# fluent/chunkio

Measured on AMD Instinct MI355X. Metric: device-resident CRC32 GB/s over N×400KB chunks; % HBM-read roofline, higher is better.
Workload: dtype u8

## Files before the change

chunkio_amd/_lib.py:

```python
import ctypes
import os
import sys

HERE = os.path.dirname(os.path.abspath(__file__))
LIB_PATH = os.environ.get("CIO_AMD_LIB") or os.path.join(HERE, "lib", "libchunkio_amd.so")

EXPORTS = (
    "crc_update",
    "cio_gpu_init", "cio_gpu_last_error", "cio_gpu_version",
    "cio_crc32_shift", "cio_crc32_combine",
    "cio_crc32_plan_create", "cio_crc32_plan_destroy", "cio_crc32_plan_exec",
    "cio_crc32_plan_exec_events", "cio_crc32_plan_bytes", "cio_crc32_plan_kernel", "cio_crc32_plan_workgroups", "cio_crc32_ring_create", "cio_crc32_ring_exec",
    "cio_crc32_ring_join", "cio_crc32_ring_destroy", "cio_crc32_batch_dev", "cio_crc32_batch_host",
    "cio_crc32_devplan_create", "cio_crc32_devplan_destroy", "cio_crc32_devplan_exec", "cio_crc32_devplan_workgroups",
    "cio_crc32_batch_host_multi", "cio_crc32_split_host_multi", "cio_crc32_batch_fd_multi", "cio_gpu_device_count", "cio_gpu_set_device", "cio_gpu_get_device", "cio_gpu_numa_node",
    "cio_gpu_pci_bus_id", "cio_gpu_plan_cache_stats",
    "cio_crc32_host_register", "cio_crc32_host_unregister", "cio_gpu_pipe_last_timing",
    "cio_crc32_cpu_max", "cio_crc32_set_cpu_max", "cio_crc32_split_route", "cio_crc32_set_split_route", "cio_crc32_split_rates", "cio_crc32_split_forget", "cio_crc32_host_threads", "cio_crc32_set_host_threads",
    "cio_crc32_route_reset",
    "cio_crc32_batch_cpu", "cio_crc32_batch_fd_cpu",
    "cio_gpu_fill_synthetic", "cio_sha1_batch_dev", "cio_sha1_batch_dev_async",
    "cio_sha1_state_init", "cio_sha1_update_batch_dev", "cio_sha1_final_batch_dev", "cio_gpu_read_stream", "cio_gpu_read_stream_grid",
    "cio_gpu_event_create", "cio_gpu_event_destroy", "cio_gpu_event_record",
    "cio_gpu_event_elapsed_ms", "cio_gpu_stream_sync",
    "cio_sha1_init", "cio_sha1_update", "cio_sha1_final", "cio_sha1_hash", "cio_sha1_to_hex",
    "cioa_SHA1_Init", "cioa_SHA1_Update", "cioa_SHA1_Final",
    "cio_file_verify_batch", "cio_file_verify_batch_multi", "cio_verify_paths", "cio_verify_paths_multi",
    "cio_file_verify_batch_dev",
    "cio_dev_writer_create", "cio_dev_writer_destroy", "cio_file_init_batch_dev", "cio_file_write_batch_dev",
    "cio_file_seal_batch_dev",
    "cio_dev_writer_create_ex", "cio_dev_writer_move_segments", "cio_file_write_metadata_batch_dev",
    "cio_file_write_at_batch_dev",
    "cio_file_read_batch_dev", "cio_file_read_packed_batch_dev", "cio_meta_cmp_batch_dev",
    "cio_file_sync_batch", "cio_file_sync_batch_multi", "cio_file_sync_batch_begin", "cio_file_sync_batch_end",
    "cioa_create", "cioa_destroy", "cioa_set_max_chunks_up", "cioa_set_realloc_size_hint",
    "cioa_enable_file_trimming", "cioa_disable_file_trimming", "cioa_get_flags", "cioa_set_devices",
    "cioa_last_chunk_error", "cioa_total_chunks", "cioa_total_chunks_up",
    "cioa_stream_create", "cioa_stream_get", "cioa_stream_size_chunks_up", "cioa_stream_chunks", "cioa_scan_stream", "cioa_scan_streams", "cioa_scan_dump",
    "cioa_chunk_open", "cioa_chunk_close", "cioa_chunk_delete", "cioa_chunk_write", "cioa_chunk_write_at",
    "cioa_chunk_sync", "cioa_chunk_sync_batch", "cioa_chunk_sync_batch_begin", "cioa_chunk_sync_batch_end",
    "cioa_chunk_get_content", "cioa_chunk_get_content_copy",
    "cioa_chunk_get_content_size", "cioa_chunk_get_content_end_pos", "cioa_chunk_is_file",
    "cioa_chunk_close_stream", "cioa_chunk_get_real_size", "cioa_chunk_hash", "cioa_chunk_lock",
    "cioa_chunk_unlock", "cioa_chunk_is_locked", "cioa_chunk_tx_begin", "cioa_chunk_tx_commit",
    "cioa_chunk_tx_rollback", "cioa_chunk_is_up", "cioa_chunk_up", "cioa_chunk_up_force",
    "cioa_chunk_up_batch", "cioa_chunk_up_force_batch", "cioa_chunk_down",
    "cioa_chunk_name", "cioa_chunk_map", "cioa_error_get", "cioa_chunk_crc_cur", "cioa_chunk_set_crc_cur",
    "cioa_meta_write", "cioa_meta_read", "cioa_meta_cmp", "cioa_meta_size", "cioa_bench_perf_write",
)

_lib = None
_hip_runtime = None

c_u64_p = ctypes.POINTER(ctypes.c_uint64)
c_u32_p = ctypes.POINTER(ctypes.c_uint32)


def _bind(lib):
    V, P = ctypes.c_void_p, ctypes.POINTER
    sig = {
        "crc_update": (ctypes.c_uint64, [ctypes.c_uint64, V, ctypes.c_size_t]),
        "cio_gpu_init": (ctypes.c_int, []),
        "cio_gpu_last_error": (ctypes.c_char_p, []),
        "cio_gpu_version": (ctypes.c_char_p, []),
        "cio_crc32_shift": (ctypes.c_uint32, [ctypes.c_uint32, ctypes.c_uint64]),
        "cio_crc32_combine": (ctypes.c_uint32, [ctypes.c_uint32, ctypes.c_uint32, ctypes.c_uint64]),
        "cio_crc32_plan_create": (ctypes.c_int, [P(V), c_u64_p, c_u64_p, ctypes.c_size_t]),
        "cio_crc32_plan_destroy": (None, [V]),
        "cio_crc32_plan_exec": (ctypes.c_int, [V, V, V, V, V]),
        "cio_crc32_plan_exec_events": (ctypes.c_int, [V, V, V, V, V, V, V]),
        "cio_crc32_plan_bytes": (ctypes.c_uint64, [V]),
        "cio_crc32_plan_kernel": (ctypes.c_char_p, [V]),
        "cio_crc32_plan_workgroups": (ctypes.c_uint32, [V]),
        "cio_crc32_ring_create": (ctypes.c_int, [ctypes.POINTER(V), ctypes.POINTER(ctypes.c_uint64),
                                                 ctypes.POINTER(ctypes.c_uint64), ctypes.c_size_t, ctypes.c_int]),
        "cio_crc32_ring_exec": (ctypes.c_int, [V, V, V, V, V]),
        "cio_crc32_ring_join": (ctypes.c_int, [V, V]),
        "cio_crc32_ring_destroy": (None, [V]),
        "cio_crc32_batch_dev": (ctypes.c_int, [V, c_u64_p, c_u64_p, V, V, ctypes.c_size_t, V]),
        "cio_crc32_devplan_create": (ctypes.c_int, [P(V), ctypes.c_size_t]),
        "cio_crc32_devplan_destroy": (None, [V]),
        "cio_crc32_devplan_exec": (ctypes.c_int, [V, V, ctypes.c_uint64, V, V, ctypes.c_size_t, V, V, V, V]),
        "cio_crc32_devplan_workgroups": (ctypes.c_uint32, [V]),
        "cio_file_verify_batch_dev": (ctypes.c_int, [V, V, ctypes.c_uint64, V, V, ctypes.c_size_t, ctypes.c_int,
                                                     V, V, V, V, V, V]),
        "cio_dev_writer_create": (ctypes.c_int, [P(V), ctypes.c_size_t]),
        "cio_dev_writer_destroy": (None, [V]),
        "cio_file_init_batch_dev": (ctypes.c_int, [V, V, ctypes.c_uint64, V, V, ctypes.c_size_t, V, ctypes.c_uint64,
                                                   V, V, ctypes.c_int, V, V, V]),
        "cio_file_write_batch_dev": (ctypes.c_int, [V, V, ctypes.c_uint64, V, V, ctypes.c_size_t, V, ctypes.c_uint64,
                                                    V, V, ctypes.c_int, V, V, V]),
        "cio_file_seal_batch_dev": (ctypes.c_int, [V, V, ctypes.c_uint64, V, V, ctypes.c_size_t, ctypes.c_int,
                                                   V, V, V]),
        "cio_dev_writer_create_ex": (ctypes.c_int, [P(V), ctypes.c_size_t, ctypes.c_int]),
        "cio_dev_writer_move_segments": (ctypes.c_uint32, [V]),
        "cio_file_write_metadata_batch_dev": (ctypes.c_int, [V, V, ctypes.c_uint64, V, V, ctypes.c_size_t, V,
                                                             ctypes.c_uint64, V, V, ctypes.c_int, V, V, V]),
        "cio_file_write_at_batch_dev": (ctypes.c_int, [V, V, ctypes.c_uint64, V, V, ctypes.c_size_t, V, V,
                                                       ctypes.c_uint64, V, V, ctypes.c_int, V, V, V]),
        "cio_file_read_batch_dev": (ctypes.c_int, [V, V, ctypes.c_uint64, V, V, ctypes.c_size_t, ctypes.c_int, V,
                                                   V, ctypes.c_uint64, V, V, ctypes.c_int, V, V, V]),
        "cio_file_read_packed_batch_dev": (ctypes.c_int, [V, V, ctypes.c_uint64, V, V, ctypes.c_size_t, ctypes.c_int,
                                                          V, V, ctypes.c_uint64, ctypes.c_uint64, ctypes.c_int, V, V,
                                                          V, V, V]),
        "cio_meta_cmp_batch_dev": (ctypes.c_int, [V, ctypes.c_uint64, V, V, ctypes.c_size_t, V, ctypes.c_uint64, V,
                                                  V, V, V, V]),
        "cio_crc32_batch_host": (ctypes.c_int, [P(V), P(ctypes.c_size_t), c_u32_p, c_u32_p,
                                                ctypes.c_size_t]),
        "cio_crc32_batch_host_multi": (ctypes.c_int, [P(V), P(ctypes.c_size_t), c_u32_p, c_u32_p,
                                                      ctypes.c_size_t, P(ctypes.c_int), ctypes.c_int]),
        "cio_crc32_split_host_multi": (ctypes.c_int, [V, ctypes.c_size_t, ctypes.c_uint32, c_u32_p,
                                                      P(ctypes.c_int), ctypes.c_int]),
        "cio_gpu_device_count": (ctypes.c_int, []),
        "cio_gpu_set_device": (ctypes.c_int, [ctypes.c_int]),
        "cio_gpu_get_device": (ctypes.c_int, []),
        "cio_gpu_numa_node": (ctypes.c_int, [ctypes.c_int]),
        "cio_gpu_pci_bus_id": (ctypes.c_int, [ctypes.c_int, ctypes.c_char_p, ctypes.c_int]),
        "cio_gpu_plan_cache_stats": (ctypes.c_int, [ctypes.POINTER(ctypes.c_uint64), ctypes.c_int]),
        "cio_crc32_host_register": (ctypes.c_int, [V, ctypes.c_size_t]),
        "cio_crc32_host_unregister": (ctypes.c_int, [V]),
        "cio_gpu_pipe_last_timing": (ctypes.c_int, [P(ctypes.c_double), ctypes.c_int]),
        "cio_crc32_cpu_max": (ctypes.c_size_t, []),
        "cio_crc32_set_cpu_max": (None, [ctypes.c_size_t]),
        "cio_crc32_split_route": (ctypes.c_int, []),
        "cio_crc32_set_split_route": (None, [ctypes.c_int]),
        "cio_crc32_split_rates": (None, [ctypes.POINTER(ctypes.c_double), ctypes.c_int]),
# ... 116 lines not shown
```

chunkio_amd/crc32.py:

```python
import ctypes

import numpy as np

from . import _lib

CRC_INIT = 0xFFFFFFFF


def crc_init():
    return CRC_INIT


def crc_finalize(crc):
    return (crc ^ 0xFFFFFFFF) & 0xFFFFFFFF


def _as_bytes(data):
    if isinstance(data, np.ndarray):
        return np.ascontiguousarray(data).view(np.uint8)
    return np.frombuffer(memoryview(data).cast("B"), dtype=np.uint8)


def crc_update(crc, data):
    buf = _as_bytes(data)
# ... 2 lines not shown


def crc32(data, seed=CRC_INIT):
    return crc_finalize(crc_update(seed, data))


def crc32_shift(raw_state, nbytes):
    return int(_lib.lib().cio_crc32_shift(raw_state & 0xFFFFFFFF, nbytes))


def crc32_combine(raw_a, raw0_b, len_b):
    return int(_lib.lib().cio_crc32_combine(raw_a & 0xFFFFFFFF, raw0_b & 0xFFFFFFFF, len_b))


def _u64_array(values):
    arr = np.ascontiguousarray(np.asarray(values, dtype=np.uint64))
    return arr, arr.ctypes.data_as(_lib.c_u64_p)


def _ptr(t):
    return None if t is None else ctypes.c_void_p(t.data_ptr())


def _stream_ptr(stream):
    if stream is None:
        import torch
        stream = torch.cuda.current_stream()
    return ctypes.c_void_p(int(stream.cuda_stream))


class Crc32Plan:

    def __init__(self, offs, lens):
        self._offs, po = _u64_array(offs)
        self._lens, pl = _u64_array(lens)
        if self._offs.shape != self._lens.shape:
            raise ValueError("offs and lens must have the same length")
        self.n = int(self._offs.size)
        handle = ctypes.c_void_p()
        _lib.check(_lib.lib().cio_crc32_plan_create(ctypes.byref(handle), po, pl, self.n),
                   "cio_crc32_plan_create")
        self._handle = handle

    @property
    def bytes(self):
        return int(_lib.lib().cio_crc32_plan_bytes(self._handle))

    @property
    def workgroups(self):
        return int(_lib.lib().cio_crc32_plan_workgroups(self._handle))

    def kernel_name(self):
        return _lib.lib().cio_crc32_plan_kernel(self._handle).decode()

    def exec(self, base, out, seeds=None, stream=None):
        _lib.check(_lib.lib().cio_crc32_plan_exec(self._handle, _ptr(base), _ptr(seeds), _ptr(out),
                                                  _stream_ptr(stream)),
                   "cio_crc32_plan_exec")

    def exec_events(self, base, out, ev_start, ev_stop, seeds=None, stream=None):
        _lib.check(_lib.lib().cio_crc32_plan_exec_events(self._handle, _ptr(base), _ptr(seeds),
                                                         _ptr(out), _stream_ptr(stream),
                                                         ev_start, ev_stop),
                   "cio_crc32_plan_exec_events")

    def close(self):
        if getattr(self, "_handle", None):
            _lib.lib().cio_crc32_plan_destroy(self._handle)
            self._handle = None

    def __del__(self):
        try:
            self.close()
        except Exception:
            pass

    def __enter__(self):
        return self

    def __exit__(self, *exc):
        self.close()


class Crc32Ring:

    def __init__(self, offs, lens, depth=2):
        self._offs, po = _u64_array(offs)
        self._lens, pl = _u64_array(lens)
        if self._offs.shape != self._lens.shape:
            raise ValueError("offs and lens must have the same length")
        self.n = int(self._offs.size)
        handle = ctypes.c_void_p()
        _lib.check(_lib.lib().cio_crc32_ring_create(ctypes.byref(handle), po, pl, self.n, int(depth)),
                   "cio_crc32_ring_create")
        self._handle = handle

    def exec(self, base, out, seeds=None, stream=None):
        _lib.check(_lib.lib().cio_crc32_ring_exec(self._handle, _ptr(base), _ptr(seeds), _ptr(out),
                                                  _stream_ptr(stream)),
                   "cio_crc32_ring_exec")

    def join(self, stream=None):
        _lib.check(_lib.lib().cio_crc32_ring_join(self._handle, _stream_ptr(stream)), "cio_crc32_ring_join")

    def close(self):
        if getattr(self, "_handle", None):
# ... 334 lines not shown
```

chunkio_amd/csrc/cio_plan.h:

```cpp
#ifndef CIOA_PLAN_H
#define CIOA_PLAN_H

#include <stddef.h>
#include <stdint.h>
#include <vector>

#include "cio_diag.h"
#include "crc32_host.h"
#include "chunkio_amd/cio_crc32_gpu.h"

namespace cioa {

constexpr int kWave = 64;
constexpr int kGran = 16;
constexpr int kSub = 4;
constexpr int kRow = kWave * kGran;
constexpr int kStep = kSub * kRow;
constexpr int kThreads = 1024;
constexpr uint32_t kWavesPerWg = kThreads / kWave;
constexpr uint32_t kWfFold = 1u, kWfPublish = 2u;
constexpr int kX8Count = 2 * kStep;
constexpr uint32_t kSliceBytes = 131072;
constexpr uint32_t kShiftBytes = 32768;
constexpr uint32_t kShiftOff = kSliceBytes;
constexpr uint32_t kLdsBytes = kSliceBytes + kShiftBytes;
constexpr int kStampWords = 16;

struct ChunkDesc {
    uint64_t a;
    uint64_t vlen;
    uint64_t g;
    uint32_t nsteps;
    uint32_t h;
    uint32_t npieces;
    uint32_t w0, w1;
    uint32_t pad;
};
static_assert(sizeof(ChunkDesc) == 48, "desc layout");

struct WaveStart {
    ChunkDesc d;
    uint32_t c;
    uint32_t pad[3];
};
static_assert(sizeof(WaveStart) == 64, "wave start layout");

struct DeviceState {
    bool ready = false;
    int cus = 0;
    uint32_t *slice = nullptr;
    uint32_t *shift = nullptr;
    uint32_t *x8 = nullptr;
    uint32_t *xinv8 = nullptr;
};

struct PlanHost {
    std::vector<ChunkDesc> desc;
    std::vector<WaveStart> ws;
    std::vector<uint32_t> tiny;
    std::vector<uint32_t> pfac;
    uint64_t S = 0, bytes = 0;
};

void plan_init(cio_crc32_plan *p, DeviceState *st, size_t n);
const char *plan_build(PlanHost &ph, const uint64_t *offs, const uint64_t *lens, size_t n, uint32_t W);
const char *plan_choose(cio_crc32_plan *p, PlanHost &ph, const uint64_t *offs, const uint64_t *lens, size_t n);

constexpr int kDevHdrS = 0, kDevHdrNtiny = 1, kDevHdrBytes = 2, kDevHdrStatus = 3, kDevHdrWords = 4;
constexpr uint32_t kPlanBlock = 1024;

struct PlanBlockSum {
    uint64_t steps, bytes;
    uint32_t ntiny, err;
};

}

struct cio_crc32_plan {
    uint32_t n = 0;
    uint64_t S = 0;
    uint32_t W = 0;
    uint32_t grid = 0;
    uint32_t ntiny = 0;
    int prio = 1;
    uint64_t ustride = 0, ua0 = 0, uvlen = 0;
    uint32_t unsteps = 0, uh = 0;
    bool small = false;
    bool ahead = false;
    bool l64 = false;
    bool l64_small = false;
    unsigned long long *stamps = nullptr;
    uint64_t bytes = 0;
    cioa::ChunkDesc *desc = nullptr;
    cioa::WaveStart *wstart = nullptr;
    uint32_t *tiny = nullptr;
    unsigned long long *partials = nullptr;
    uint32_t *counters = nullptr;
    uint32_t *pfac = nullptr;
    cioa::DeviceState *st = nullptr;
};

#endif
```

chunkio_amd/csrc/crc32_gpu.hip:

```cpp

#include <hip/hip_runtime.h>
#include <stdint.h>
#include <algorithm>
#include <type_traits>

#include "cio_gpu_internal.h"
#include "crc_wave.h"

using namespace cioa;

namespace {


constexpr uint32_t cx_multmodp(uint32_t a, uint32_t b)
{
    uint32_t p = 0;
    for (int i = 31; i >= 0; --i) {
        if ((a >> i) & 1u) {
            p ^= b;
        }
        b = (b & 1u) ? (b >> 1) ^ CIOA_POLY : (b >> 1);
    }
    return p;
}
// ... 782 lines not shown
        t_arrived = __builtin_amdgcn_s_memrealtime();
    }
    tiny_chunks(lds, lb_lo, base, desc, tiny, seeds, out, cid, ntiny, wave, lane, W);
    __syncthreads();
    if (STAMPS) {
        t_bar1 = __builtin_amdgcn_s_memrealtime();
    }
    uint32_t *slot = reinterpret_cast<uint32_t *>(lds);
    if (lane == 0) {
        slot[tid >> 6] = pub;
    }
    __syncthreads();
    if (STAMPS) {
        t_bar2 = __builtin_amdgcn_s_memrealtime();
    }
    if (wfl & kWfFold) {
        const uint32_t nb = (wfl >> 8) & 0xffu;
        uint32_t a = 0;
        if (lane < kWavesPerWg && lane >= kWavesPerWg - nb) {
            a = slot[(tid >> 6) + lane - kWavesPerWg];
        }
        a = wave_xor(a) ^ fold_own;
        if (lane == 0) {
            out[cid ? cid[c0] : c0] = a;
        }
    }
    if (STAMPS) {
        t_folded = __builtin_amdgcn_s_memrealtime();
    }
    if (STAMPS && lane == 0) {
        uint32_t hw_id, xcc_id;
        asm volatile("s_getreg_b32 %0, hwreg(HW_REG_HW_ID)" : "=s"(hw_id));
        asm volatile("s_getreg_b32 %0, hwreg(HW_REG_XCC_ID)" : "=s"(xcc_id));
        stamps[kStampWords * wave + 0] = t_entry;
        stamps[kStampWords * wave + 1] = t_tables;
        stamps[kStampWords * wave + 2] = t_stream;
        stamps[kStampWords * wave + 3] = __builtin_amdgcn_s_memrealtime();
        stamps[kStampWords * wave + 4] = hw_id;
        stamps[kStampWords * wave + 5] = xcc_id;
        stamps[kStampWords * wave + 6] = t_first;
        stamps[kStampWords * wave + 7] = t_mid;
        stamps[kStampWords * wave + 8] = t_issued;
        stamps[kStampWords * wave + 9] = t_wt[0];
        stamps[kStampWords * wave + 10] = t_wt[1];
        stamps[kStampWords * wave + 11] = t_step1;
        stamps[kStampWords * wave + 12] = t_arrived;
        stamps[kStampWords * wave + 13] = t_bar1;
        stamps[kStampWords * wave + 14] = t_bar2;
        stamps[kStampWords * wave + 15] = t_folded;
    }
}


struct SmallRegs {
    uint4 q[kSub];
    uint32_t inv;
    uint32_t seed;
};

__device__ __forceinline__ uint4 mask_tail(uint4 v, uint32_t bs, uint32_t vlen)
{
    uint32_t w[4] = {v.x, v.y, v.z, v.w};
#pragma unroll
    for (int i = 0; i < 4; ++i) {
        const uint32_t b = bs + 4u * i;
        const uint32_t nb = b >= vlen ? 0u : min(vlen - b, 4u);
        w[i] &= nb >= 4u ? ~0u : ((1u << (8u * nb)) - 1u);
    }
    return make_uint4(w[0], w[1], w[2], w[3]);
}

template <bool UNI, bool SEEDS, bool L64 = false>
__global__ void __launch_bounds__(kThreads, 1)
crc32_small_kernel(const uint8_t *base, uint64_t ustride, uint64_t ua0, uint64_t uvlen, uint32_t uh,
                   uint32_t W, uint32_t n, uint32_t ntiny, const uint32_t *__restrict__ g_x8,
                   const ChunkDesc *__restrict__ desc,
                   const uint32_t *__restrict__ tiny, const uint32_t *__restrict__ seeds, uint32_t *out,
                   const uint32_t *__restrict__ g_xinv8)
{
    __shared__ __attribute__((aligned(16))) char lds[kLdsBytes];
    const uint32_t tid = threadIdx.x;
    const uint32_t wave = __builtin_amdgcn_readfirstlane(blockIdx.x * (kThreads / kWave) + (tid >> 6));
    const uint32_t lane = tid & 63u;
    const uint32_t lb_lo = (lane & kSliceRepMask) << 2;
    const uint32_t lb_hi = lb_lo | 0x10000u;
    const uint32_t lrep = (lane & kShiftRepMask) << 2;
    const uint32_t c0 = __builtin_amdgcn_readfirstlane((uint32_t) split_point(wave, n, W));
    const uint32_t c1 = __builtin_amdgcn_readfirstlane((uint32_t) split_point((uint64_t) wave + 1, n, W));
    const uint32_t lbyte = lane * kGran;
    const uint32_t loff = L64 ? 64u * (lane & 15u) + 16u * (lane >> 4) : lbyte;
    const uint32_t *const seeds_p = seeds ? seeds : g_x8;

    auto geom = [&](uint32_t c, uint64_t &a, uint32_t &vlen, uint32_t &h, bool &live) {
        if (UNI) {
            a = ua0 + (uint64_t) c * ustride;
            vlen = (uint32_t) uvlen;
            h = uh;
            asm volatile("" : "+s"(vlen), "+s"(h));
            live = true;
        } else {
            const ChunkDesc d = desc[c];
            a = d.a;
            vlen = (uint32_t) d.vlen;
            h = d.h;
            live = d.nsteps != 0;
        }
// ... 95 lines not shown
            }
            st = block16(lds, lb_lo, lb_hi, 0u, r.q[0]);
#pragma unroll
            for (int q = 1; q < kSub; ++q) {
                st = L64 ? block16(lds, lb_lo, lb_hi, st, r.q[q])
                         : shift_block16(lds, lb_lo, lb_hi, lrep, st, r.q[q]);
            }
        }
        uint32_t inv = inv_u;
        if (!UNI) {
            asm volatile("v_mov_b32 %0, %1" : "=v"(inv) : "v"(cur.inv));
        }
        issue(cur, c + 1);
        if (live) {
            uint32_t x = col[0] & (0u - (st & 1u));
#pragma unroll
            for (int j = 1; j < 32; ++j) {
                x = xor_and(x, 0u - ((st >> j) & 1u), col[j]);
            }
            uint32_t crc = wave_xor(x);
            if (vlen != (uint32_t) kStep) {
                asm volatile("" : "+v"(inv));
                crc = multmodp(inv, crc);
            }
            if (lane == 0) {
                out[c] = crc;
            }
        }
    };
    const uint32_t slot_group = __builtin_amdgcn_readfirstlane((tid >> 6) >> 2);
    for (uint32_t c = c0; c < c1; ++c) {
        rotate_prio(slot_group, c - c0);
        chunk(cur, c);
    }
    __builtin_amdgcn_s_setprio(0);
    tiny_chunks(lds, lb_lo, base, desc, tiny, seeds, out, nullptr, ntiny, wave, lane, W);
}


}

extern "C" {

int cioa_debug_stamps(const cio_crc32_plan *p, unsigned long long *host, size_t cap)
{
    if (!p || !p->stamps) {
        return 0;
    }
    const size_t n = std::min(cap, (size_t) p->W * kStampWords);
    if (hipMemcpy(host, p->stamps, n * sizeof(unsigned long long), hipMemcpyDeviceToHost) != hipSuccess) {
        return 0;
    }
    return (int) p->W;
}

}

using StreamKernel = decltype(&crc32_stream_kernel<false, 1, false>);

static StreamKernel select_kernel(int prio, bool stamps, bool uniform, bool ahead, bool l64)
{
    if (ahead) {
        if (l64) {
            if (stamps) {
                return crc32_stream_kernel<true, 1, true, true, true>;
            }
            return prio ? crc32_stream_kernel<false, 1, true, true, true>
                        : crc32_stream_kernel<false, 0, true, true, true>;
        }
        return prio ? crc32_stream_kernel<false, 1, true, true> : crc32_stream_kernel<false, 0, true, true>;
    }
    if (l64 && !stamps) {
        return prio ? crc32_stream_kernel<false, 1, false, false, true>
                    : crc32_stream_kernel<false, 0, false, false, true>;
    }
    switch ((prio ? 4 : 0) + (stamps ? 2 : 0) + (uniform ? 1 : 0)) {
    case 0: return crc32_stream_kernel<false, 0, false>;
    case 1: return crc32_stream_kernel<false, 0, true>;
    case 2: return crc32_stream_kernel<true, 0, false>;
    case 3: return crc32_stream_kernel<true, 0, true>;
    case 4: return crc32_stream_kernel<false, 1, false>;
    case 5: return crc32_stream_kernel<false, 1, true>;
    case 6: return crc32_stream_kernel<true, 1, false>;
    default: return crc32_stream_kernel<true, 1, true>;
    }
}


int cioa::plan_exec_impl(const cio_crc32_plan *p, const void *dev_base, const uint32_t *dev_seeds,
                         uint32_t *dev_out, const uint32_t *cid, hipStream_t s,
                         hipEvent_t ev0, hipEvent_t ev1)
{
    if (!p) {
        return fail("cio_crc32_plan_exec: null plan");
    }
    if (p->n == 0) {
        return CIO_OK;
    }
    if (!dev_base || !dev_out) {
        return fail("cio_crc32_plan_exec: null buffer");
    }
    const DeviceState *st = p->st;
    if (ev0) {
        HIP_TRY(hipEventRecord(ev0, s), "hipEventRecord");
    }
    if (p->small && !cid) {
        auto sk = p->l64_small ? (p->unsteps ? (dev_seeds ? crc32_small_kernel<true, true, true>
                                                    : crc32_small_kernel<true, false, true>)
                                       : (dev_seeds ? crc32_small_kernel<false, true, true>
                                                    : crc32_small_kernel<false, false, true>))
                         : (p->unsteps ? (dev_seeds ? crc32_small_kernel<true, true> : crc32_small_kernel<true, false>)
                                       : (dev_seeds ? crc32_small_kernel<false, true>
                                                    : crc32_small_kernel<false, false>));
        hipLaunchKernelGGL(sk, dim3(p->grid), dim3(kThreads), 0, s,
                           reinterpret_cast<const uint8_t *>(dev_base), p->ustride, p->ua0, p->uvlen, p->uh,
                           p->W, p->n, p->ntiny, st->x8, p->desc, p->tiny, dev_seeds, dev_out, st->xinv8);
        HIP_TRY(hipGetLastError(), "crc32_small_kernel launch");
        if (ev1) {
            HIP_TRY(hipEventRecord(ev1, s), "hipEventRecord");
        }
        return CIO_OK;
    }
    auto kern = select_kernel(p->prio, p->stamps != nullptr, p->unsteps != 0, p->ahead && (!p->stamps || p->l64),
                              p->l64);
    hipLaunchKernelGGL(kern, dim3(p->grid), dim3(kThreads), 0, s,
                       reinterpret_cast<const uint8_t *>(dev_base), p->S, p->ustride, p->ua0, p->uvlen,
                       p->W, p->unsteps, p->uh, p->n, p->desc, p->wstart, p->tiny,
                       dev_seeds, dev_out, cid, p->partials, p->counters, st->slice, st->shift,
                       st->x8, p->pfac, p->ntiny, p->stamps);
    HIP_TRY(hipGetLastError(), "crc32_stream_kernel launch");
    if (ev1) {
        HIP_TRY(hipEventRecord(ev1, s), "hipEventRecord");
    }
    return CIO_OK;
}

int cioa::devplan_crc_launch(const cio_crc32_plan *p, const unsigned long long *hdr, const void *dev_base,
                             const uint32_t *dev_seeds, uint32_t *dev_out, size_t n, hipStream_t s)
{
    const DeviceState *st = p->st;
    StreamKernel kern = p->l64 ? (p->prio ? crc32_stream_kernel<false, 1, false, false, true, true>
                                          : crc32_stream_kernel<false, 0, false, false, true, true>)
                               : (p->prio ? crc32_stream_kernel<false, 1, false, false, false, true>
                                          : crc32_stream_kernel<false, 0, false, false, false, true>);
    hipLaunchKernelGGL(kern, dim3(p->grid), dim3(kThreads), 0, s,
                       reinterpret_cast<const uint8_t *>(dev_base), (uint64_t) 0, (uint64_t) 0, (uint64_t) 0,
                       (uint64_t) 0, p->W, 0u, 0u, (uint32_t) n, p->desc, p->wstart, p->tiny,
                       dev_seeds, dev_out, (const uint32_t *) nullptr, p->partials, p->counters, st->slice,
                       st->shift, st->x8, p->pfac, 0u, const_cast<unsigned long long *>(hdr));
    HIP_TRY(hipGetLastError(), "crc32_stream_kernel (device-planned) launch");
    return CIO_OK;
}
```

chunkio_amd/csrc/crc_plan.cpp:

```cpp

#include <stdint.h>
#include <stdlib.h>
#include <string.h>
#include <algorithm>
#include <vector>

#include "cio_plan.h"

namespace cioa {

void plan_init(cio_crc32_plan *p, DeviceState *st, size_t n)
{
    p->st = st;
    p->n = (uint32_t) n;
    if (const char *r = cioa_diag_getenv("CIO_GPU_PRIO")) {
        const int v = atoi(r);
        p->prio = (v == 0) ? 0 : 1;
    }
    p->l64 = true;
    p->l64_small = false;
    if (const char *r = cioa_diag_getenv("CIO_GPU_L64")) {
        p->l64 = p->l64_small = atoi(r) != 0;
    }
    p->grid = (uint32_t) st->cus;
// ... 148 lines not shown
    p->uh = ph.desc[0].h;
    p->unsteps = ph.desc[0].nsteps;
}

}

const char *plan_choose(cio_crc32_plan *p, PlanHost &ph, const uint64_t *offs, const uint64_t *lens, size_t n)
{
    if (const char *err = plan_build(ph, offs, lens, n, p->W)) {
        return err;
    }
    plan_uniform(p, offs, lens, n, ph);
    auto small_batch = [&ph, n] { return ph.S > 0 && ph.S == (uint64_t) n - ph.tiny.size(); };
    bool oversub = false;
    if (!cioa_diag_getenv("CIO_GPU_GRID") && ph.S >= 1024ull * p->W && 4ull * p->W <= 65536 &&
        !small_batch()) {
        PlanHost ph4;
        if (plan_build(ph4, offs, lens, n, 4 * p->W) == nullptr) {
            p->grid *= 4;
            p->W *= 4;
            oversub = true;
            ph = std::move(ph4);
        }
    }
    {
        const char *r = cioa_diag_getenv("CIO_GPU_ANTICAMP");
        const bool on = !(r && atoi(r) == 0);
        const char *mx = cioa_diag_getenv("CIO_GPU_ANTICAMP_MAX");
        const uint64_t wmax = mx ? strtoull(mx, nullptr, 10) : small_batch() ? 128 : 64;
        const uint64_t w = p->W ? ph.S / p->W : 0;
        const bool any_grid = r && atoi(r) == 2;
        if (on && (!oversub || any_grid) && !cioa_diag_getenv("CIO_GPU_GRID") && p->grid % 32 == 0 && ph.S % p->W == 0 &&
            w % 16 == 0 &&
            w > 0 && w <= wmax) {
            const uint32_t g2 = p->grid / 32 * 31;
            PlanHost ph2;
            if (plan_build(ph2, offs, lens, n, g2 * (kThreads / kWave)) == nullptr) {
                p->grid = g2;
                p->W = g2 * (kThreads / kWave);
                ph = std::move(ph2);
            }
        }
    }
    p->S = ph.S;
    p->bytes = ph.bytes;
    p->ntiny = (uint32_t) ph.tiny.size();
    p->ahead = p->unsteps != 0 && p->uh == 0 && p->uvlen % kStep == 0;
    bool short_ranges = p->S <= 64ull * p->W;
    if (const char *r = cioa_diag_getenv("CIO_GPU_AHEAD")) {
        short_ranges = atoi(r) != 0;
    }
    p->ahead = p->ahead && short_ranges;

    p->small = small_batch();
    if (const char *r = cioa_diag_getenv("CIO_GPU_SMALL")) {
        p->small = p->small && atoi(r) != 0;
    }
    return nullptr;
}

}

using namespace cioa;

extern "C" {

int cioa_debug_plan_layout(const uint64_t *offs, const uint64_t *lens, size_t n, uint32_t W,
                           uint32_t *chunk_words, uint32_t *wave_flags)
{
    PlanHost ph;
    if (plan_build(ph, offs, lens, n, W) != nullptr) {
        return -1;
    }
    for (size_t i = 0; i < n; i++) {
        chunk_words[3 * i + 0] = ph.desc[i].w0;
        chunk_words[3 * i + 1] = ph.desc[i].w1;
        chunk_words[3 * i + 2] = ph.desc[i].npieces;
    }
    const size_t nslots = (size_t) W + n + 1;
    for (uint32_t w = 0; w < W; w++) {
        wave_flags[w] = ph.pfac[nslots + w];
    }
    return 0;
}

int cioa_debug_plan_image(const uint64_t *offs, const uint64_t *lens, size_t n, uint32_t W, void *desc,
                          void *wstart, uint32_t *tiny, uint32_t *pfac, uint64_t *hdr)
{
    PlanHost ph;
    if (plan_build(ph, offs, lens, n, W) != nullptr) {
        return -1;
    }
    memcpy(desc, ph.desc.data(), n * sizeof(ChunkDesc));
    memcpy(wstart, ph.ws.data(), (size_t) W * sizeof(WaveStart));
    if (!ph.tiny.empty()) {
        memcpy(tiny, ph.tiny.data(), ph.tiny.size() * sizeof(uint32_t));
    }
    memcpy(pfac, ph.pfac.data(), ph.pfac.size() * sizeof(uint32_t));
    hdr[kDevHdrS] = ph.S;
    hdr[kDevHdrNtiny] = ph.tiny.size();
    hdr[kDevHdrBytes] = ph.bytes;
    hdr[kDevHdrStatus] = 0;
    return 0;
}

int cioa_debug_plan_choice(const uint64_t *offs, const uint64_t *lens, size_t n, int cus, uint32_t *out_words)
{
    if (cus < 1 || n >= 0xffffffffull) {
        return -1;
    }
    DeviceState st;
    st.cus = cus;
    cio_crc32_plan p;
    PlanHost ph;
    plan_init(&p, &st, n);
    if (plan_choose(&p, ph, offs, lens, n) != nullptr) {
        return -1;
    }
    const uint64_t ntiny = p.ntiny;
    const uint32_t words[11] = {p.grid, p.W, p.small, p.ahead, p.unsteps, p.l64, p.l64_small,
                                (uint32_t) p.S, (uint32_t) (p.S >> 32), (uint32_t) ntiny, (uint32_t) (ntiny >> 32)};
    memcpy(out_words, words, sizeof(words));
    return 0;
}

}
```

chunkio_amd/csrc/gpu_runtime.hip:

```cpp

#include <hip/hip_runtime.h>
#include <stdint.h>
#include <string.h>
#include <stdio.h>
#include <stdlib.h>
#include <memory>
#include <mutex>
#include <vector>
#include <string>
#include <algorithm>

#include "cio_gpu_internal.h"

using namespace cioa;

namespace cioa {

thread_local std::string g_err;

int fail(const char *what, hipError_t e)
{
    char buf[512];
    if (e != hipSuccess) {
        snprintf(buf, sizeof(buf), "%s: %s", what, hipGetErrorString(e));
// ... 32 lines not shown
    if (!st.ready) {
        hipDeviceProp_t prop;
        HIP_TRY(hipGetDeviceProperties(&prop, dev), "hipGetDeviceProperties");
        if (strncmp(prop.gcnArchName, "gfx950", 6) != 0) {
            char msg[256];
            snprintf(msg, sizeof(msg), "chunkio_amd kernels are built for gfx950, device is %s",
                     prop.gcnArchName);
            return fail(msg);
        }
        st.cus = prop.multiProcessorCount;
        static uint32_t slice[4][256], shift[4][256];
        std::vector<uint32_t> x8(kX8Count);
        cioa_gen_slice4(slice);
        cioa_gen_shift_table(shift, (uint64_t) (kStep - kGran));
        cioa_gen_xpow8_table(x8.data(), kX8Count, 1);
        HIP_TRY(hipMalloc(&st.slice, sizeof(slice)), "hipMalloc(slice)");
        HIP_TRY(hipMalloc(&st.shift, sizeof(shift)), "hipMalloc(shift)");
        HIP_TRY(hipMalloc(&st.x8, kX8Count * sizeof(uint32_t)), "hipMalloc(x8)");
        HIP_TRY(hipMemcpy(st.slice, slice, sizeof(slice), hipMemcpyHostToDevice), "upload slice");
        HIP_TRY(hipMemcpy(st.shift, shift, sizeof(shift), hipMemcpyHostToDevice), "upload shift");
        HIP_TRY(hipMemcpy(st.x8, x8.data(), kX8Count * sizeof(uint32_t), hipMemcpyHostToDevice),
                "upload x8");
        std::vector<uint32_t> xinv8(kStep);
        uint32_t xm8 = 0x80000000u;
        for (int i = 0; i < 8; ++i) {
            xm8 = cioa_multmodp(xm8, (CIOA_POLY << 1) | 1u);
        }
        xinv8[0] = 0x80000000u;
        for (int d = 1; d < kStep; ++d) {
            xinv8[d] = cioa_multmodp(xinv8[d - 1], xm8);
        }
        HIP_TRY(hipMalloc(&st.xinv8, kStep * sizeof(uint32_t)), "hipMalloc(xinv8)");
        HIP_TRY(hipMemcpy(st.xinv8, xinv8.data(), kStep * sizeof(uint32_t), hipMemcpyHostToDevice),
                "upload xinv8");
        st.ready = true;
    }
    *out = &st;
    return CIO_OK;
}

}

extern "C" {

const char *cio_gpu_last_error(void)
{
    return g_err.c_str();
}

const char *cio_gpu_version(void)
{
#define CIO_STR2(x) #x
#define CIO_STR(x) CIO_STR2(x)
    return "chunkio_amd crc32 v9 gfx950 stream(l64-lanes permlane-transpose issue-ahead<=64steps pre-shift prio-rotate "
           "coalesced-nt division-free-start slice4-lds32x perm direct-whole preshifted-partials wg-lds-fold "
           "head-align=" CIO_STR(CIO_HEAD_ALIGN) ") "
           "small(4x16B dpp-reduce bitop3-fold prio-rotate) "
           "host(nt-staging graduated-groups pread-bounce multi-device vpclmul-crc_update small-batch-route) "
           "sha1(2-schedule-waves 4-block-handover continuation)";
}

int cio_gpu_init(void)
{
    DeviceState *st;
    return device_state(&st);
}

void cio_crc32_plan_destroy(cio_crc32_plan *p)
{
    if (!p) {
        return;
    }
    (void) hipFree(p->desc);
    (void) hipFree(p->wstart);
    (void) hipFree(p->tiny);
    (void) hipFree(p->partials);
    (void) hipFree(p->counters);
    (void) hipFree(p->pfac);
    (void) hipFree(p->stamps);
    delete p;
}

int cio_crc32_plan_create(cio_crc32_plan **out, const uint64_t *offs, const uint64_t *lens, size_t n)
{
    if (!out || (n && (!offs || !lens))) {
        return fail("cio_crc32_plan_create: null argument");
    }
    if (n >= 0xffffffffull) {
        return fail("cio_crc32_plan_create: too many chunks");
    }
    *out = nullptr;
    DeviceState *st;
    if (device_state(&st) != CIO_OK) {
        return CIO_ERROR;
    }
    cio_crc32_plan *p = new cio_crc32_plan();
    plan_init(p, st, n);
    PlanHost ph;
    if (const char *err = plan_choose(p, ph, offs, lens, n)) {
        delete p;
        return fail(err);
    }
    if (const char *r = cioa_diag_getenv("CIO_GPU_STAMPS")) {
        if (atoi(r) > 0 && hipMalloc(&p->stamps, (size_t) p->W * kStampWords * sizeof(unsigned long long)) != hipSuccess) {
            p->stamps = nullptr;
        }
    }
    hipError_t e;
    const size_t npart = ph.pfac.size();
    if ((e = hipMalloc(&p->desc, ph.desc.size() * sizeof(ChunkDesc))) != hipSuccess ||
        (e = hipMalloc(&p->wstart, ph.ws.size() * sizeof(WaveStart))) != hipSuccess ||
        (e = hipMalloc(&p->tiny, std::max<size_t>(1, ph.tiny.size()) * sizeof(uint32_t))) != hipSuccess ||
        (e = hipMalloc(&p->partials, npart * sizeof(unsigned long long))) != hipSuccess ||
        (e = hipMalloc(&p->counters, std::max<size_t>(1, n) * sizeof(uint32_t))) != hipSuccess ||
        (e = hipMalloc(&p->pfac, npart * sizeof(uint32_t))) != hipSuccess ||
        (e = hipMemcpy(p->desc, ph.desc.data(), ph.desc.size() * sizeof(ChunkDesc), hipMemcpyHostToDevice)) != hipSuccess ||
        (e = hipMemcpy(p->wstart, ph.ws.data(), ph.ws.size() * sizeof(WaveStart), hipMemcpyHostToDevice)) != hipSuccess ||
        (ph.tiny.size() && (e = hipMemcpy(p->tiny, ph.tiny.data(), ph.tiny.size() * sizeof(uint32_t), hipMemcpyHostToDevice)) != hipSuccess) ||
        (e = hipMemset(p->partials, 0, npart * sizeof(unsigned long long))) != hipSuccess ||
        (e = hipMemset(p->counters, 0, std::max<size_t>(1, n) * sizeof(uint32_t))) != hipSuccess ||
        (e = hipMemcpy(p->pfac, ph.pfac.data(), npart * sizeof(uint32_t), hipMemcpyHostToDevice)) != hipSuccess) {
        cio_crc32_plan_destroy(p);
        return fail("cio_crc32_plan_create: device allocation/upload", e);
    }
    *out = p;
    return CIO_OK;
}

uint64_t cio_crc32_plan_bytes(const cio_crc32_plan *p)
{
    return p ? p->bytes : 0;
}

uint32_t cio_crc32_plan_workgroups(const cio_crc32_plan *p)
{
    return p ? p->grid : 0;
}

const char *cio_crc32_plan_kernel(const cio_crc32_plan *p)
{
    return (p && p->small) ? "crc32_small_kernel" : "crc32_stream_kernel";
}

int cio_crc32_plan_exec_events(const cio_crc32_plan *p, const void *dev_base,
                               const uint32_t *dev_seeds, uint32_t *dev_out, void *stream,
                               void *ev_piece_start, void *ev_piece_stop)
{
    return plan_exec_impl(p, dev_base, dev_seeds, dev_out, nullptr,
                          reinterpret_cast<hipStream_t>(stream),
                          reinterpret_cast<hipEvent_t>(ev_piece_start),
                          reinterpret_cast<hipEvent_t>(ev_piece_stop));
}

int cio_crc32_plan_exec(const cio_crc32_plan *p, const void *dev_base, const uint32_t *dev_seeds,
                        uint32_t *dev_out, void *stream)
{
    return plan_exec_impl(p, dev_base, dev_seeds, dev_out, nullptr,
                          reinterpret_cast<hipStream_t>(stream));
}

int cio_crc32_batch_dev(const void *dev_base, const uint64_t *offs, const uint64_t *lens,
                        const uint32_t *dev_seeds, uint32_t *dev_out, size_t n, void *stream)
{
    cio_crc32_plan *p = nullptr;
    if (cio_crc32_plan_create(&p, offs, lens, n) != CIO_OK) {
        return CIO_ERROR;
    }
    int rc = cio_crc32_plan_exec(p, dev_base, dev_seeds, dev_out, stream);
    if (rc == CIO_OK) {
        hipError_t e = hipStreamSynchronize(reinterpret_cast<hipStream_t>(stream));
        if (e != hipSuccess) {
            rc = fail("cio_crc32_batch_dev: stream sync", e);
        }
    }
    cio_crc32_plan_destroy(p);
    return rc;
}

struct cio_crc32_ring {
    std::vector<cio_crc32_plan *> plans;
    std::vector<hipStream_t> streams;
    std::vector<hipEvent_t> ready, done;
    std::vector<bool> pending;
    unsigned next = 0;
    int dev = 0;
};

struct RingDevice {
    int prev = -1;
    hipError_t e = hipSuccess;
    explicit RingDevice(int dev)
    {
        if ((e = hipGetDevice(&prev)) == hipSuccess && prev != dev) {
            e = hipSetDevice(dev);
// ... 146 lines not shown
```

include/chunkio_amd/cio_crc32_gpu.h:

```cpp
#ifndef CIO_CRC32_GPU_H
#define CIO_CRC32_GPU_H

#include <stddef.h>
#include <stdint.h>
#include <chunkio_amd/cio_sha1_state.h>

#ifdef __cplusplus
extern "C" {
#endif

#ifndef CIO_OK
#define CIO_OK       0
#define CIO_ERROR   -1
#endif


int cio_gpu_init(void);

int cio_gpu_device_count(void);
int cio_gpu_set_device(int dev);
int cio_gpu_get_device(void);

int cio_gpu_numa_node(int dev);

int cio_gpu_pci_bus_id(int dev, char *buf, int len);

const char *cio_gpu_last_error(void);

const char *cio_gpu_version(void);


uint32_t cio_crc32_shift(uint32_t raw_state, uint64_t nbytes);

uint32_t cio_crc32_combine(uint32_t raw_a, uint32_t raw0_b, uint64_t len_b);


typedef struct cio_crc32_plan cio_crc32_plan;

int  cio_crc32_plan_create(cio_crc32_plan **plan, const uint64_t *offs,
                           const uint64_t *lens, size_t n);
void cio_crc32_plan_destroy(cio_crc32_plan *plan);

int  cio_crc32_plan_exec(const cio_crc32_plan *plan, const void *dev_base,
                         const uint32_t *dev_seeds, uint32_t *dev_out,
                         void *stream);

int  cio_crc32_plan_exec_events(const cio_crc32_plan *plan, const void *dev_base,
                                const uint32_t *dev_seeds, uint32_t *dev_out,
                                void *stream, void *ev_piece_start,
                                void *ev_piece_stop);

uint64_t cio_crc32_plan_bytes(const cio_crc32_plan *plan);

const char *cio_crc32_plan_kernel(const cio_crc32_plan *plan);

typedef struct cio_crc32_ring cio_crc32_ring;
int  cio_crc32_ring_create(cio_crc32_ring **ring, const uint64_t *offs, const uint64_t *lens, size_t n, int depth);
int  cio_crc32_ring_exec(cio_crc32_ring *ring, const void *dev_base, const uint32_t *dev_seeds, uint32_t *dev_out,
                         void *stream);
int  cio_crc32_ring_join(cio_crc32_ring *ring, void *stream);
void cio_crc32_ring_destroy(cio_crc32_ring *ring);

uint32_t cio_crc32_plan_workgroups(const cio_crc32_plan *plan);

int  cio_crc32_batch_dev(const void *dev_base, const uint64_t *offs,
                         const uint64_t *lens, const uint32_t *dev_seeds,
                         uint32_t *dev_out, size_t n, void *stream);

typedef struct cio_crc32_devplan cio_crc32_devplan;

#define CIO_DEVPLAN_E_BOUNDS           1
#define CIO_DEVPLAN_E_CHUNK_TOO_LARGE  2
#define CIO_DEVPLAN_E_BATCH_TOO_LARGE  4

int  cio_crc32_devplan_create(cio_crc32_devplan **plan, size_t max_chunks);
void cio_crc32_devplan_destroy(cio_crc32_devplan *plan);

int  cio_crc32_devplan_exec(cio_crc32_devplan *plan, const void *dev_base, uint64_t dev_bytes,
                            const uint64_t *dev_offs, const uint64_t *dev_lens, size_t n,
                            const uint32_t *dev_seeds, uint32_t *dev_out,
                            uint32_t *dev_status, void *stream);

uint32_t cio_crc32_devplan_workgroups(const cio_crc32_devplan *plan);


int  cio_crc32_batch_host(const void *const *bufs, const size_t *lens,
                          const uint32_t *seeds, uint32_t *out_raw, size_t n);

int  cio_crc32_batch_host_multi(const void *const *bufs, const size_t *lens,
                                const uint32_t *seeds, uint32_t *out_raw, size_t n,
                                const int *devices, int ndev);

int  cio_crc32_split_host_multi(const void *buf, size_t len, uint32_t seed, uint32_t *out_raw,
                                const int *devices, int ndev);

int  cio_crc32_batch_fd_multi(const int *fds, const uint64_t *foffs, const size_t *lens,
                              const uint32_t *seeds, uint32_t *out_raw, size_t n,
                              const int *devices, int ndev);

int  cio_crc32_host_register(const void *p, size_t len);
int  cio_crc32_host_unregister(const void *p);

int  cio_gpu_pipe_last_timing(double *out, int n);

int  cio_gpu_plan_cache_stats(uint64_t *out, int n);


// ... 60 lines not shown
```

Before: 6289.

## Add wave-aligned CRC32 kernel for uniform chunk layouts with precomputed shift factors

Adds a specialized kernel used when every chunk splits evenly into a power-of-two number of wave pieces with equal step counts. Each wave derives its chunk and piece from its index, so it skips the generic per-wave start descriptors. It combines partial CRCs with precomputed per-lane shift factors through an LDS fold within the workgroup instead of global partials and counters. The path is on by default when the plan's conditions hold and adds a separate factor table upload, plus a new code path that must match the generic kernel's results.

```diff
diff --git a/chunkio_amd/_lib.py b/chunkio_amd/_lib.py
--- a/chunkio_amd/_lib.py
+++ b/chunkio_amd/_lib.py
@@ -10,7 +10,7 @@
     "cio_gpu_init", "cio_gpu_last_error", "cio_gpu_version",
     "cio_crc32_shift", "cio_crc32_combine",
     "cio_crc32_plan_create", "cio_crc32_plan_destroy", "cio_crc32_plan_exec",
-    "cio_crc32_plan_exec_events", "cio_crc32_plan_bytes", "cio_crc32_plan_kernel", "cio_crc32_plan_workgroups", "cio_crc32_ring_create", "cio_crc32_ring_exec",
+    "cio_crc32_plan_exec_events", "cio_crc32_plan_bytes", "cio_crc32_plan_kernel", "cio_crc32_plan_aligned", "cio_crc32_plan_workgroups", "cio_crc32_ring_create", "cio_crc32_ring_exec",
     "cio_crc32_ring_join", "cio_crc32_ring_destroy", "cio_crc32_batch_dev", "cio_crc32_batch_host",
     "cio_crc32_devplan_create", "cio_crc32_devplan_destroy", "cio_crc32_devplan_exec", "cio_crc32_devplan_workgroups",
     "cio_crc32_batch_host_multi", "cio_crc32_split_host_multi", "cio_crc32_batch_fd_multi", "cio_gpu_device_count", "cio_gpu_set_device", "cio_gpu_get_device", "cio_gpu_numa_node",
@@ -72,6 +72,7 @@
         "cio_crc32_plan_bytes": (ctypes.c_uint64, [V]),
         "cio_crc32_plan_kernel": (ctypes.c_char_p, [V]),
         "cio_crc32_plan_workgroups": (ctypes.c_uint32, [V]),
+        "cio_crc32_plan_aligned": (ctypes.c_int, [V]),
         "cio_crc32_ring_create": (ctypes.c_int, [ctypes.POINTER(V), ctypes.POINTER(ctypes.c_uint64),
                                                  ctypes.POINTER(ctypes.c_uint64), ctypes.c_size_t, ctypes.c_int]),
         "cio_crc32_ring_exec": (ctypes.c_int, [V, V, V, V, V]),
diff --git a/chunkio_amd/crc32.py b/chunkio_amd/crc32.py
--- a/chunkio_amd/crc32.py
+++ b/chunkio_amd/crc32.py
@@ -78,6 +78,10 @@
 
     def kernel_name(self):
         return _lib.lib().cio_crc32_plan_kernel(self._handle).decode()
+
+    @property
+    def aligned(self):
+        return bool(_lib.lib().cio_crc32_plan_aligned(self._handle))
 
     def exec(self, base, out, seeds=None, stream=None):
         _lib.check(_lib.lib().cio_crc32_plan_exec(self._handle, _ptr(base), _ptr(seeds), _ptr(out),
diff --git a/chunkio_amd/csrc/cio_plan.h b/chunkio_amd/csrc/cio_plan.h
--- a/chunkio_amd/csrc/cio_plan.h
+++ b/chunkio_amd/csrc/cio_plan.h
@@ -59,6 +59,7 @@
     std::vector<WaveStart> ws;
     std::vector<uint32_t> tiny;
     std::vector<uint32_t> pfac;
+    std::vector<uint32_t> afac;
     uint64_t S = 0, bytes = 0;
 };
 
@@ -89,6 +90,9 @@
     bool ahead = false;
     bool l64 = false;
     bool l64_small = false;
+    bool aligned = false;
+    uint32_t aq = 0, alg2p = 0;
+    uint32_t *afac = nullptr;
     unsigned long long *stamps = nullptr;
     uint64_t bytes = 0;
     cioa::ChunkDesc *desc = nullptr;
diff --git a/chunkio_amd/csrc/crc32_gpu.hip b/chunkio_amd/csrc/crc32_gpu.hip
--- a/chunkio_amd/csrc/crc32_gpu.hip
+++ b/chunkio_amd/csrc/crc32_gpu.hip
@@ -858,6 +858,187 @@
 }
 
 
+template <bool STAMPS = false>
+__global__ void __launch_bounds__(kThreads, 1)
+crc32_aligned_kernel(const uint8_t *base, uint64_t ustride, uint64_t ua0, uint32_t q, uint32_t lgp,
+                     const uint32_t *__restrict__ afac, const uint32_t *__restrict__ seeds, uint32_t *out,
+                     const uint32_t *__restrict__ cid, unsigned long long *stamps)
+{
+    __shared__ __attribute__((aligned(16))) char lds[kLdsBytes];
+    const uint32_t tid = threadIdx.x;
+    unsigned long long t_entry = 0, t_tables = 0, t_stream = 0, t_first = 0, t_mid = 0, t_issued = 0;
+    unsigned long long t_wt[2] = {0, 0}, t_step1 = 0, t_bar1 = 0, t_bar2 = 0, t_folded = 0;
+    if (STAMPS) {
+        t_entry = __builtin_amdgcn_s_memrealtime();
+    }
+    const uint32_t wslot = __builtin_amdgcn_readfirstlane(tid >> 6);
+    const uint32_t wave = blockIdx.x * (uint32_t) kWavesPerWg + wslot;
+    const uint32_t lane = tid & 63u;
+    const uint32_t np = 1u << lgp;
+    const uint32_t c = wave >> lgp, piece = wave & (np - 1u);
+    const uint8_t *cbase = base + (ua0 + (uint64_t) c * ustride + (uint64_t) (piece * q * (uint32_t) kStep));
+
+    StepRegs cur, nxt;
+    load_step64(cur, cbase, 0, lane);
+    __builtin_amdgcn_sched_barrier(0);
+    const uint32_t fac = afac[piece * (uint32_t) kWave + lane];
+    __builtin_amdgcn_sched_barrier(0);
+    if (STAMPS) {
+        t_issued = __builtin_amdgcn_s_memrealtime();
+    }
+    const uint32_t lb_lo = (lane & kSliceRepMask) << 2;
+    const uint32_t lb_hi = lb_lo | 0x10000u;
+    const uint32_t lrep = (lane & kShiftRepMask) << 2;
+    const uint32_t slot_group = wslot >> 2;
+    {
+        uint32_t tab_v[kE], tab_sv[kE];
+        table_entries<cx_xpow8n(kStep - 64)>(__builtin_amdgcn_readfirstlane(tid >> 8), tid & 255u, tab_v[0],
+                                             tab_sv[0]);
+        write_tables<STAMPS>(lds, tid, tab_v, tab_sv, t_wt);
+    }
+    __syncthreads();
+    if (STAMPS) {
+        t_tables = __builtin_amdgcn_s_memrealtime();
+    }
+
+    const bool first_piece = piece == 0, final_piece = piece == np - 1u;
+    uint32_t oc = c;
+    if (cid && (first_piece || final_piece)) {
+        oc = cid[c];
+    }
+    uint32_t seed = 0;
+    if (first_piece) {
+        seed = seeds ? seeds[oc] : 0xffffffffu;
+    }
+    auto landed = [](StepRegs &r) {
+        asm volatile("" : "+v"(r.q[0].x), "+v"(r.q[0].y), "+v"(r.q[0].z), "+v"(r.q[0].w),
+                          "+v"(r.q[1].x), "+v"(r.q[1].y), "+v"(r.q[1].z), "+v"(r.q[1].w),
+                          "+v"(r.q[2].x), "+v"(r.q[2].y), "+v"(r.q[2].z), "+v"(r.q[2].w),
+                          "+v"(r.q[3].x), "+v"(r.q[3].y), "+v"(r.q[3].z), "+v"(r.q[3].w));
+    };
+    landed(cur);
+    cur.q[0].x ^= lane == 0 ? seed : 0u;
+    if (STAMPS) {
+        t_first = __builtin_amdgcn_s_memrealtime();
+    }
+
+    uint32_t s0 = 0;
+    uint32_t col[32];
+    auto half = [&](uint32_t it, StepRegs &use, StepRegs &fill, auto refill, auto first) {
+        rotate_prio(slot_group, it);
+        landed(use);
+        if (decltype(refill)::value) {
+            load_step64(fill, cbase, it + 1, lane);
+        }
+        if (decltype(first)::value) {
+            col[31] = fac;
+#pragma unroll
+            for (int j = 30; j >= 0; --j) {
+                col[j] = (col[j + 1] >> 1) ^ (CIOA_POLY & (0u - (col[j + 1] & 1u)));
+            }
+#pragma unroll
+            for (int j = 0; j < 32; j += 8) {
+                asm volatile("" : "+v"(col[j]), "+v"(col[j + 1]), "+v"(col[j + 2]), "+v"(col[j + 3]),
+                                  "+v"(col[j + 4]), "+v"(col[j + 5]), "+v"(col[j + 6]), "+v"(col[j + 7]));
+            }
+        }
+        const uint32_t h0 = step_shift(lds, lrep, s0);
+        transpose64(use);
+        uint32_t st = block16(lds, lb_lo, lb_hi, h0, use.q[0]);
+#pragma unroll
+        for (int k = 1; k < kSub; ++k) {
+            st = block16(lds, lb_lo, lb_hi, st, use.q[k]);
+        }
+        s0 = st;
+        if (STAMPS && it == 0) {
+            t_step1 = __builtin_amdgcn_s_memrealtime();
+        }
+        if (STAMPS && it == q / 2) {
+            t_mid = __builtin_amdgcn_s_memrealtime();
+        }
+    };
+    using Refill = std::true_type;
+    using NoRefill = std::false_type;
+    using First = std::true_type;
+    using Later = std::false_type;
+    if (q == 1) {
+        half(0, cur, nxt, NoRefill(), First());
+    } else {
+        half(0, cur, nxt, Refill(), First());
+        uint32_t it = 1;
+        for (; it + 2 < q; it += 2) {
+            half(it, nxt, cur, Refill(), Later());
+            half(it + 1, cur, nxt, Refill(), Later());
+        }
+        if (q - it == 2) {
+            half(it, nxt, cur, Refill(), Later());
+            half(it + 1, cur, nxt, NoRefill(), Later());
+        } else {
+            half(it, nxt, cur, NoRefill(), Later());
+        }
+    }
+    __builtin_amdgcn_s_setprio(0);
+    if (STAMPS) {
+        t_stream = __builtin_amdgcn_s_memrealtime();
+    }
+
+    uint32_t acc[4] = {0u, 0u, 0u, 0u};
+#pragma unroll
+    for (int j = 0; j < 32; ++j) {
+        acc[j & 3] = xor_and(acc[j & 3], 0u - ((s0 >> j) & 1u), col[j]);
+    }
+    const uint32_t contrib = wave_xor(xor3(acc[0], acc[1], acc[2]) ^ acc[3]);
+
+    __syncthreads();
+    if (STAMPS) {
+        t_bar1 = __builtin_amdgcn_s_memrealtime();
+    }
+    uint32_t *slot = reinterpret_cast<uint32_t *>(lds);
+    if (!final_piece && lane == 0) {
+        slot[wslot] = contrib;
+    }
+    __syncthreads();
+    if (STAMPS) {
+        t_bar2 = __builtin_amdgcn_s_memrealtime();
+    }
+    if (final_piece) {
+        uint32_t x = 0;
+        if (lane < np - 1u) {
+            x = slot[wslot - (np - 1u) + lane];
+        }
+        x = wave_xor(x) ^ contrib;
+        if (lane == 0) {
+            out[oc] = x;
+        }
+    }
+    if (STAMPS) {
+        t_folded = __builtin_amdgcn_s_memrealtime();
+    }
+    if (STAMPS && lane == 0) {
+        uint32_t hw_id, xcc_id;
+        asm volatile("s_getreg_b32 %0, hwreg(HW_REG_HW_ID)" : "=s"(hw_id));
+        asm volatile("s_getreg_b32 %0, hwreg(HW_REG_XCC_ID)" : "=s"(xcc_id));
+        unsigned long long *ws = stamps + (size_t) kStampWords * wave;
+        ws[0] = t_entry;
+        ws[1] = t_tables;
+        ws[2] = t_stream;
+        ws[3] = __builtin_amdgcn_s_memrealtime();
+        ws[4] = hw_id;
+        ws[5] = xcc_id;
+        ws[6] = t_first;
+        ws[7] = t_mid;
+        ws[8] = t_issued;
+        ws[9] = t_wt[0];
+        ws[10] = t_wt[1];
+        ws[11] = t_step1;
+        ws[12] = t_stream;
+        ws[13] = t_bar1;
+        ws[14] = t_bar2;
+        ws[15] = t_folded;
+    }
+}
+
+
 struct SmallRegs {
     uint4 q[kSub];
     uint32_t inv;
@@ -1059,6 +1240,12 @@
         return 0;
     }
     return (int) p->W;
+}
+
+int cioa_debug_plan_exec_cid(const cio_crc32_plan *p, const void *dev_base, const uint32_t *dev_seeds,
+                             uint32_t *dev_out, const uint32_t *dev_cid, void *stream)
+{
+    return plan_exec_impl(p, dev_base, dev_seeds, dev_out, dev_cid, reinterpret_cast<hipStream_t>(stream));
 }
 
 }
@@ -1128,6 +1315,16 @@
         }
         return CIO_OK;
     }
+    if (p->aligned) {
+        auto ak = p->stamps ? crc32_aligned_kernel<true> : crc32_aligned_kernel<false>;
+        hipLaunchKernelGGL(ak, dim3(p->grid), dim3(kThreads), 0, s, reinterpret_cast<const uint8_t *>(dev_base),
+                           p->ustride, p->ua0, p->aq, p->alg2p, p->afac, dev_seeds, dev_out, cid, p->stamps);
+        HIP_TRY(hipGetLastError(), "crc32_aligned_kernel launch");
+        if (ev1) {
+            HIP_TRY(hipEventRecord(ev1, s), "hipEventRecord");
+        }
+        return CIO_OK;
+    }
     auto kern = select_kernel(p->prio, p->stamps != nullptr, p->unsteps != 0, p->ahead && (!p->stamps || p->l64),
                               p->l64);
     hipLaunchKernelGGL(kern, dim3(p->grid), dim3(kThreads), 0, s,
diff --git a/chunkio_amd/csrc/crc_plan.cpp b/chunkio_amd/csrc/crc_plan.cpp
--- a/chunkio_amd/csrc/crc_plan.cpp
+++ b/chunkio_amd/csrc/crc_plan.cpp
@@ -224,6 +224,29 @@
     }
     p->ahead = p->ahead && short_ranges;
 
+    p->aligned = false;
+    ph.afac.clear();
+    {
+        const char *r = cioa_diag_getenv("CIO_GPU_ALIGNED");
+        const bool on = !(r && atoi(r) == 0);
+        const uint64_t q = p->W ? p->S / p->W : 0;
+        if (on && p->ahead && p->l64 && p->prio && p->ntiny == 0 && p->grid == (uint32_t) p->st->cus &&
+            q >= 1 && q <= 64 && p->S == q * p->W && p->unsteps % q == 0) {
+            const uint64_t np = p->unsteps / q;
+            if (np == 2 || np == 4 || np == 8 || np == 16) {
+                p->aligned = true;
+                p->aq = (uint32_t) q;
+                p->alg2p = np == 2 ? 1 : np == 4 ? 2 : np == 8 ? 3 : 4;
+                ph.afac.resize(np * kWave);
+                for (uint64_t i = 0; i < np; i++) {
+                    for (uint64_t l = 0; l < (uint64_t) kWave; l++) {
+                        ph.afac[i * kWave + l] = cioa_xpow8n(q * kStep * (np - 1 - i) + 64 * (kWave - 1 - l));
+                    }
+                }
+            }
+        }
+    }
+
     p->small = small_batch();
     if (const char *r = cioa_diag_getenv("CIO_GPU_SMALL")) {
         p->small = p->small && atoi(r) != 0;
@@ -296,4 +319,23 @@
     return 0;
 }
 
-}
+int cioa_debug_plan_aligned(const uint64_t *offs, const uint64_t *lens, size_t n, int cus, uint32_t *out_words)
+{
+    if (cus < 1 || n >= 0xffffffffull) {
+        return -1;
+    }
+    DeviceState st;
+    st.cus = cus;
+    cio_crc32_plan p;
+    PlanHost ph;
+    plan_init(&p, &st, n);
+    if (plan_choose(&p, ph, offs, lens, n) != nullptr) {
+        return -1;
+    }
+    out_words[0] = p.aligned;
+    out_words[1] = p.aligned ? p.aq : 0;
+    out_words[2] = p.aligned ? 1u << p.alg2p : 0;
+    return 0;
+}
+
+}
diff --git a/chunkio_amd/csrc/gpu_runtime.hip b/chunkio_amd/csrc/gpu_runtime.hip
--- a/chunkio_amd/csrc/gpu_runtime.hip
+++ b/chunkio_amd/csrc/gpu_runtime.hip
@@ -108,7 +108,7 @@
 {
 #define CIO_STR2(x) #x
 #define CIO_STR(x) CIO_STR2(x)
-    return "chunkio_amd crc32 v9 gfx950 stream(l64-lanes permlane-transpose issue-ahead<=64steps pre-shift prio-rotate "
+    return "chunkio_amd crc32 v9 gfx950 stream(l64-lanes permlane-transpose issue-ahead<=64steps wave-aligned pre-shift prio-rotate "
            "coalesced-nt division-free-start slice4-lds32x perm direct-whole preshifted-partials wg-lds-fold "
            "head-align=" CIO_STR(CIO_HEAD_ALIGN) ") "
            "small(4x16B dpp-reduce bitop3-fold prio-rotate) "
@@ -133,6 +133,7 @@
     (void) hipFree(p->partials);
     (void) hipFree(p->counters);
     (void) hipFree(p->pfac);
+    (void) hipFree(p->afac);
     (void) hipFree(p->stamps);
     delete p;
 }
@@ -175,7 +176,10 @@
         (ph.tiny.size() && (e = hipMemcpy(p->tiny, ph.tiny.data(), ph.tiny.size() * sizeof(uint32_t), hipMemcpyHostToDevice)) != hipSuccess) ||
         (e = hipMemset(p->partials, 0, npart * sizeof(unsigned long long))) != hipSuccess ||
         (e = hipMemset(p->counters, 0, std::max<size_t>(1, n) * sizeof(uint32_t))) != hipSuccess ||
-        (e = hipMemcpy(p->pfac, ph.pfac.data(), npart * sizeof(uint32_t), hipMemcpyHostToDevice)) != hipSuccess) {
+        (e = hipMemcpy(p->pfac, ph.pfac.data(), npart * sizeof(uint32_t), hipMemcpyHostToDevice)) != hipSuccess ||
+        (p->aligned && ((e = hipMalloc(&p->afac, ph.afac.size() * sizeof(uint32_t))) != hipSuccess ||
+                        (e = hipMemcpy(p->afac, ph.afac.data(), ph.afac.size() * sizeof(uint32_t),
+                                       hipMemcpyHostToDevice)) != hipSuccess))) {
         cio_crc32_plan_destroy(p);
         return fail("cio_crc32_plan_create: device allocation/upload", e);
     }
@@ -196,6 +200,11 @@
 const char *cio_crc32_plan_kernel(const cio_crc32_plan *p)
 {
     return (p && p->small) ? "crc32_small_kernel" : "crc32_stream_kernel";
+}
+
+int cio_crc32_plan_aligned(const cio_crc32_plan *p)
+{
+    return (p && p->aligned) ? 1 : 0;
 }
 
 int cio_crc32_plan_exec_events(const cio_crc32_plan *p, const void *dev_base,
diff --git a/include/chunkio_amd/cio_crc32_gpu.h b/include/chunkio_amd/cio_crc32_gpu.h
--- a/include/chunkio_amd/cio_crc32_gpu.h
+++ b/include/chunkio_amd/cio_crc32_gpu.h
@@ -53,6 +53,8 @@
 uint64_t cio_crc32_plan_bytes(const cio_crc32_plan *plan);
 
 const char *cio_crc32_plan_kernel(const cio_crc32_plan *plan);
+
+int cio_crc32_plan_aligned(const cio_crc32_plan *plan);
 
 typedef struct cio_crc32_ring cio_crc32_ring;
 int  cio_crc32_ring_create(cio_crc32_ring **ring, const uint64_t *offs, const uint64_t *lens, size_t n, int depth);
```

After: 6640, median of 6. +5.6%, better.
